# RRr89/Shared_SIMD_Scan

Measured on AMD Instinct MI355X. Metric: scanned values/sec + achieved HBM GB/s, 1e9 x 9-bit column (equality scan, bitmap + hit count out), higher is better.
Workload: dtype u32; 1 GPU; scan_eq ONE 1e+09x9bit column in 1 row-range shard(s) of <= 1000000000 rows, column=mod5, key=3; rows_total=1000000000, bits=9, parallelism=row-range shards x1

## Files before the change

shared_simd_scan_amd/csrc/kernels/scan.hpp:

```cpp
#pragma once

#include "tile.hpp"

namespace mi355 {

template <int C, int VPL> struct TileCtx {
    using G = ScanGeom<C, VPL>;
    uint64_t n, ntiles, nfull, data_bytes;
    uint32_t llc_inv, llc_lim;
    __device__ __forceinline__ TileCtx(uint64_t n_, uint32_t llc_inv_ = 0, uint32_t llc_lim_ = 0) : n(n_), llc_inv(llc_inv_), llc_lim(llc_lim_)
    {
        ntiles = (n + G::TILE_VALUES - 1) / G::TILE_VALUES;
        nfull = n / G::TILE_VALUES;
        data_bytes = (n * C + 7) / 8;
    }
    template <int AUX> __device__ __forceinline__ void issue(const uint8_t *packed, uint64_t t, uint8_t *lds_wave, int lane) const
    {
        if constexpr (AUX != 0) {
            if (llc_inv != 0 && (uint32_t)((t * G::TILE_BYTES) >> kLlcGranuleShift) * llc_inv <= llc_lim) {
                issue_as<0>(packed, t, lds_wave, lane);
                return;
            }
        }
        issue_as<AUX>(packed, t, lds_wave, lane);
    }
    template <int AUX> __device__ __forceinline__ void issue_as(const uint8_t *packed, uint64_t t, uint8_t *lds_wave, int lane) const
    {
        const uint8_t *src = packed + t * G::TILE_BYTES;
        if (t < nfull)
            dma_tile_full<G::TILE_BYTES, AUX>(src, lds_wave, lane);
        else
            dma_tile_partial<G::TILE_BYTES, AUX>(src, data_bytes - t * G::TILE_BYTES, lds_wave, lane);
    }
    __device__ __forceinline__ uint32_t finish_tail(uint64_t t, uint32_t (&v)[VPL / 32], uint8_t *dst, uint64_t byte_stride, int lane,
                                                    bool store = true) const
    {
        const int64_t left = (int64_t)(n - t * G::TILE_VALUES) - (int64_t)lane * VPL;
        const int valid = left >= VPL ? VPL : (left <= 0 ? 0 : (int)left);
        const int nbytes = (valid + 7) / 8;
        uint32_t cnt = 0;
#pragma unroll
        for (int j = 0; j < VPL / 32; j++) {
            v[j] &= tail_mask(valid, j);
            cnt += __builtin_popcount(v[j]);
#pragma unroll
            for (int b = 0; b < 4; b++)
                if (store && 4 * j + b < nbytes) dst[(uint64_t)(4 * j + b) * byte_stride] = (uint8_t)(v[j] >> (8 * b));
        }
        return cnt;
    }
};

template <int C, int VPL, int K> constexpr int burst_occ()
{
    using G = ScanGeom<C, VPL>;
    constexpr int mask_bytes = (K * G::BITMAP_BYTES + 1023) / 1024 * 1024;
    constexpr int table = narrow_k<C>() ? (1 << (narrow_k<C>() * C)) : 16;
    constexpr int lds = (160 * 1024) / (4 * (G::LDS_BYTES + mask_bytes) + table + 64);
    constexpr int cap = narrow_k<C>() ? 4 : 8;
    return lds > cap ? cap : (lds < 1 ? 1 : lds);
}

template <int C, int MODE, int AUX_, int VPL, int K>
__global__ __launch_bounds__(kBlockThreads, (burst_occ<C, VPL, K>())) void scan_burst_kernel(ScanArgs a)
{
    using G = ScanGeom<C, VPL>;
    static_assert(MODE == kModeEq || MODE == kModeRange, "MODE");
    constexpr int WORDS = G::WORDS;
    constexpr int AUX = AUX_ & 15;
    constexpr int NTS = store_policy_of(AUX_);
    __shared__ __attribute__((aligned(16))) uint8_t lds[kWavesPerBlock][G::LDS_BYTES];
    constexpr int LK = narrow_k<C>();
    __shared__ __attribute__((aligned(16))) uint8_t nlut[LK ? (1 << (LK * C)) : 16];
    constexpr int MASK_DMA = (K * G::BITMAP_BYTES + 1023) / 1024;
    __shared__ __attribute__((aligned(16))) uint8_t mlds[kWavesPerBlock][MASK_DMA * 1024];

    const int lane = threadIdx.x & 63;
    const int wave = __builtin_amdgcn_readfirstlane(threadIdx.x >> 6);
    uint8_t *lds_wave = lds[wave];
    uint8_t *mlds_wave = mlds[wave];
    const TileCtx<C, VPL> tc(a.n, a.llc_inv, a.llc_lim);
    const uint64_t nchunks = (tc.ntiles + K - 1) / K;
    const uint64_t stride = (uint64_t)gridDim.x * kWavesPerBlock;
    uint64_t chunk = (uint64_t)blockIdx.x * kWavesPerBlock + wave;

    uint32_t key[2] = {a.key[0], a.key[1]};
    uint32_t hits = 0;
    uint8_t *const out_lane = a.out + lane * (WORDS * 4);
    const bool store = a.out != nullptr;
    const uint8_t *const mask = a.and_mask;
    const uint32_t mop = a.mask_op, inv = a.invert;
    auto combine = [mop](uint32_t r, uint32_t m) -> uint32_t {
        return mop == 0 ? (r & m) : mop == 1 ? (r | m) : mop == 2 ? (r ^ m) : (m & ~r);
    };

    uint32_t res[K][WORDS];
    uint64_t pend_chunk = 0;
    int pend_n = 0;

    if (chunk < nchunks) tc.template issue<AUX>(a.packed, chunk * K, lds_wave, lane);
    if constexpr (LK > 0) {
        constexpr uint32_t fmask = (1u << C) - 1u;
        for (uint32_t e = threadIdx.x; e < (1u << (LK * C)); e += kBlockThreads) {
            uint32_t m = 0;
#pragma unroll
            for (int j = 0; j < LK; j++) {
                const uint32_t f = (e >> (j * C)) & fmask;
                const bool hit = (MODE == kModeRange) ? (f - key[0]) <= key[1] : f == key[0];
                m |= (hit ? 1u : 0u) << j;
            }
            nlut[e] = (uint8_t)m;
        }
        __syncthreads();
    }

    while (chunk < nchunks) {
        const uint64_t tfirst = chunk * K;
        int nfull_here = 0;
#pragma unroll
        for (int k = 0; k < K; k++) {
            const uint64_t tile = tfirst + k;
            if (tile < tc.ntiles) {
                asm volatile("s_waitcnt vmcnt(0)" ::: "memory");
                uint32_t w[G::LANE_DWORDS];
                read_lane_data<C, VPL>(lds_wave, lane, w);
                uint32_t mcur[WORDS];
                if (k > 0 && mask) {
#pragma unroll
                    for (int j = 0; j < WORDS; j++) mcur[j] = ((const uint32_t *)(mlds_wave + k * G::BITMAP_BYTES + lane * (WORDS * 4)))[j];
                }
                asm volatile("s_waitcnt lgkmcnt(0)" ::: "memory");
                if (k == 0) {
                    if (pend_n && store) {
                        uint8_t *dst = out_lane + pend_chunk * K * G::BITMAP_BYTES;
#pragma unroll
                        for (int q = 0; q < K; q++)
                            if (q < pend_n) store_words<WORDS, NTS>(dst + q * G::BITMAP_BYTES, res[q]);
                    }
                    pend_n = 0;
                    if (mask) {
                        const uint64_t mbytes = (tc.nfull > tfirst ? (tc.nfull - tfirst < K ? tc.nfull - tfirst : K) : 0) * G::BITMAP_BYTES;
                        const uint8_t *src = mask + tfirst * G::BITMAP_BYTES;
#pragma unroll
                        for (int q = 0; q < MASK_DMA; q++) {
                            const uint32_t o = q * 1024 + lane * 16;
                            if (o < mbytes) __builtin_amdgcn_global_load_lds(MI355_GPTR(src + o), MI355_LPTR(mlds_wave + q * 1024), 16, 0, 0);
                        }
                    }
                }
                const uint64_t next = (k + 1 < K && tile + 1 < tc.ntiles) ? tile + 1 : (chunk + stride) * K;
                const bool have_next = next < tc.ntiles && (k + 1 < K || chunk + stride < nchunks);
                if (have_next) tc.template issue<AUX>(a.packed, next, lds_wave, lane);
                uint32_t r1[1][WORDS];
                if constexpr (LK > 0) {
                    decode_words_narrow<C, VPL, LK, 0, G::LANE_DWORDS>(w, r1, nlut);
                } else {
                    const uint32_t key8[kMaxKeysPerPass] = {key[0], key[1], 0, 0, 0, 0, 0, 0};
                    decode_words<C, VPL, 0, 1, MODE, G::LANE_DWORDS>(w, r1, key8);
                }
#pragma unroll
                for (int j = 0; j < WORDS; j++) r1[0][j] ^= inv;
                if (tile < tc.nfull) {
                    if (mask) {
                        if (k == 0) {
                            if (have_next && next < tc.nfull)
                                asm volatile("s_waitcnt vmcnt(%0)" ::"n"(G::DMA_INSTRS) : "memory");
                            else
                                asm volatile("s_waitcnt vmcnt(0)" ::: "memory");
#pragma unroll
                            for (int j = 0; j < WORDS; j++) mcur[j] = ((const uint32_t *)(mlds_wave + lane * (WORDS * 4)))[j];
                            asm volatile("s_waitcnt lgkmcnt(0)" ::: "memory");
                        }
#pragma unroll
                        for (int j = 0; j < WORDS; j++) r1[0][j] = combine(r1[0][j], mcur[j]);
                    }
#pragma unroll
                    for (int j = 0; j < WORDS; j++) {
                        hits += __builtin_popcount(r1[0][j]);
                        res[k][j] = r1[0][j];
                    }
                    nfull_here = k + 1;
                } else {
                    if (mask) {
                        const uint8_t *mp = mask + tile * G::BITMAP_BYTES + lane * (WORDS * 4);
                        const int64_t left = (int64_t)(tc.n - tile * G::TILE_VALUES) - (int64_t)lane * VPL;
                        const int nbytes = left <= 0 ? 0 : (int)((left >= VPL ? VPL : left) + 7) / 8;
#pragma unroll
                        for (int j = 0; j < WORDS; j++) {
                            uint32_t m = 0;
#pragma unroll
                            for (int b = 0; b < 4; b++)
                                if (4 * j + b < nbytes) m |= (uint32_t)mp[4 * j + b] << (8 * b);
                            r1[0][j] = combine(r1[0][j], m);
                        }
                    }
                    hits += tc.finish_tail(tile, r1[0], out_lane + tile * G::BITMAP_BYTES, 1, lane, store);
                }
            }
        }
        pend_chunk = chunk;
        pend_n = nfull_here;
        chunk += stride;
    }
    if (pend_n && store) {
        uint8_t *dst = out_lane + pend_chunk * K * G::BITMAP_BYTES;
#pragma unroll
        for (int q = 0; q < K; q++)
            if (q < pend_n) store_words<WORDS, NTS>(dst + q * G::BITMAP_BYTES, res[q]);
    }
    if (a.hits) hits_add(a, 0, wave_sum(hits), lane);
    hits_finalize(a, 1, lane);
}

template <int C, int AUX_, int VPL>
__global__ __launch_bounds__(kBlockThreads, (burst_occ<C, VPL, 1>() > 1 ? burst_occ<C, VPL, 1>() / 2 : 1)) void scan2_kernel(ScanArgs a)
{
    using G = ScanGeom<C, VPL>;
    constexpr int WORDS = G::WORDS;
    constexpr int AUX = AUX_ & 15;
    constexpr int NTS = store_policy_of(AUX_);
    __shared__ __attribute__((aligned(16))) uint8_t lds[kWavesPerBlock][2][G::LDS_BYTES];

    const int lane = threadIdx.x & 63;
    const int wave = __builtin_amdgcn_readfirstlane(threadIdx.x >> 6);
    uint8_t *lds1 = lds[wave][0], *lds2 = lds[wave][1];
    const TileCtx<C, VPL> tc(a.n);
    const uint64_t stride = (uint64_t)gridDim.x * kWavesPerBlock;
    uint64_t tile = (uint64_t)blockIdx.x * kWavesPerBlock + wave;
    const uint32_t k1[kMaxKeysPerPass] = {a.key[0], a.key[1], 0, 0, 0, 0, 0, 0};
    const uint32_t k2[kMaxKeysPerPass] = {a.key2[0], a.key2[1], 0, 0, 0, 0, 0, 0};
    const uint32_t inv1 = a.invert, inv2 = a.invert2, mop = a.mask_op;
    auto combine = [mop](uint32_t p2, uint32_t p1) -> uint32_t {
        return mop == 0 ? (p2 & p1) : mop == 1 ? (p2 | p1) : mop == 2 ? (p2 ^ p1) : (p1 & ~p2);
    };
    uint32_t hits = 0;
    uint8_t *const out_lane = a.out + lane * (WORDS * 4);
    const bool store = a.out != nullptr;
    uint32_t res[WORDS];
    uint64_t prev = ~0ull;

    auto issue = [&](uint64_t t) {
        tc.template issue<AUX>(a.packed, t, lds1, lane);
        tc.template issue<AUX>(a.packed2, t, lds2, lane);
    };
    if (tile < tc.ntiles) issue(tile);
    while (tile < tc.ntiles) {
        asm volatile("s_waitcnt vmcnt(0)" ::: "memory");
        uint32_t w1[G::LANE_DWORDS], w2[G::LANE_DWORDS];
        read_lane_data<C, VPL>(lds1, lane, w1);
        read_lane_data<C, VPL>(lds2, lane, w2);
        asm volatile("s_waitcnt lgkmcnt(0)" ::: "memory");
        if (prev != ~0ull && store) store_words<WORDS, NTS>(out_lane + prev * G::BITMAP_BYTES, res);
        const uint64_t next = tile + stride;
        if (next < tc.ntiles) issue(next);
        uint32_t r1[1][WORDS], r2[1][WORDS];
        decode_words<C, VPL, 0, 1, kModeRange, G::LANE_DWORDS>(w1, r1, k1);
        decode_words<C, VPL, 0, 1, kModeRange, G::LANE_DWORDS>(w2, r2, k2);
#pragma unroll
        for (int j = 0; j < WORDS; j++) res[j] = combine(r2[0][j] ^ inv2, r1[0][j] ^ inv1);
        if (tile < tc.nfull) {
#pragma unroll
            for (int j = 0; j < WORDS; j++) hits += __builtin_popcount(res[j]);
            prev = tile;
        } else {
            hits += tc.finish_tail(tile, res, out_lane + tile * G::BITMAP_BYTES, 1, lane, store);
            prev = ~0ull;
        }
        tile = next;
    }
    if (prev != ~0ull && store) store_words<WORDS, NTS>(out_lane + prev * G::BITMAP_BYTES, res);
    if (a.hits) hits_add(a, 0, wave_sum(hits), lane);
    hits_finalize(a, 1, lane);
}

__device__ __forceinline__ void transpose4x4_bytes(const uint32_t (&r)[4], uint32_t (&c)[4])
{
    const uint32_t t0 = __builtin_amdgcn_perm(r[1], r[0], 0x05010400u);
    const uint32_t t1 = __builtin_amdgcn_perm(r[1], r[0], 0x07030602u);
    const uint32_t t2 = __builtin_amdgcn_perm(r[3], r[2], 0x05010400u);
    const uint32_t t3 = __builtin_amdgcn_perm(r[3], r[2], 0x07030602u);
    c[0] = __builtin_amdgcn_perm(t2, t0, 0x05040100u);
    c[1] = __builtin_amdgcn_perm(t2, t0, 0x07060302u);
    c[2] = __builtin_amdgcn_perm(t3, t1, 0x05040100u);
    c[3] = __builtin_amdgcn_perm(t3, t1, 0x07060302u);
}

}
```

shared_simd_scan_amd/csrc/kernels/tile.hpp:

```cpp
#pragma once

#include <hip/hip_runtime.h>
#include <stdint.h>

namespace mi355 {

typedef uint32_t u32x4 __attribute__((ext_vector_type(4)));
typedef uint32_t u32x2 __attribute__((ext_vector_type(2)));

#define MI355_GPTR(p) ((const __attribute__((address_space(1))) void *)(p))
#define MI355_LPTR(p) ((__attribute__((address_space(3))) void *)(p))

constexpr int kWavesPerBlock = 4;
constexpr int kBlockThreads = kWavesPerBlock * 64;
constexpr int kMaxKeysPerPass = 8;
constexpr int kMaxKeys = 1024;

template <int C, int VPL> struct ScanGeom {
    static_assert(VPL == 32 || VPL == 64 || VPL == 128, "VPL");
    static constexpr int WORDS = VPL / 32;
    static constexpr int LANE_DWORDS = VPL * C / 32;
    static constexpr int LANE_BYTES = LANE_DWORDS * 4;
    static constexpr int TILE_VALUES = 64 * VPL;
    static constexpr int TILE_BYTES = 64 * LANE_BYTES;
    static constexpr int DMA_INSTRS = (TILE_BYTES + 1023) / 1024;
    static constexpr int LDS_BYTES = DMA_INSTRS * 1024;
    static constexpr int BITMAP_BYTES = TILE_VALUES / 8;
    static constexpr int OCC_LDS = (160 * 1024) / (4 * LDS_BYTES + 64);
    static constexpr int OCC = OCC_LDS >= 8 ? 8 : (OCC_LDS < 1 ? 1 : OCC_LDS);
};

enum ScanMode { kModeEq = 0, kModeRange = 1, kModeShared = 2 };

template <int C> constexpr int narrow_k() { return C == 1 ? 8 : (C <= 3 ? 4 : (C <= 5 ? 3 : (C <= 7 ? 2 : 0))); }

template <int C, int VPL, int MODE> constexpr int scan_occ()
{
    constexpr int lds = ScanGeom<C, VPL>::OCC;
    if (MODE != 2 && C <= 7) {
        const int with_table = (160 * 1024) / (4 * ScanGeom<C, VPL>::LDS_BYTES + (1 << (narrow_k<C>() * C)) + 64);
        return with_table > 4 ? 4 : (with_table < 1 ? 1 : with_table);
    }
    return MODE == 2 ? (lds > 4 ? 4 : lds) : lds;
}

constexpr int scan_vpl(int C, int MODE)
{
    if (MODE == kModeShared) return 64;
    return C <= 16 ? 128 : 64;
}

struct ScanArgs {
    const uint8_t *packed;
    uint64_t n;
    uint8_t *out;
    uint64_t out_stride;
    unsigned long long *hits;
    unsigned long long *scratch;
    const int32_t *keys_dev;
    uint32_t key[kMaxKeysPerPass];
    uint32_t nkeys;
    uint32_t layout;
    const uint8_t *and_mask;
    uint32_t invert;
    uint32_t mask_op;
    uint32_t flags;
    const uint8_t *packed2;
    uint32_t key2[2];
    uint32_t invert2;
    unsigned long long *tile_state;
    uint64_t *rowids;
    uint64_t capacity;
    uint64_t first_row;
    uint32_t llc_d;
    uint32_t llc_inv, llc_lim;
};
constexpr int kLlcGranuleShift = 16;
inline void llc_set(ScanArgs &a, uint32_t d)
{
    a.llc_d = d;
    a.llc_inv = 0;
    a.llc_lim = 0;
    if (d == 0) return;
    uint32_t inv = d;
    for (int i = 0; i < 5; i++) inv *= 2u - d * inv;
    a.llc_inv = inv;
    a.llc_lim = 0xffffffffu / d;
}

template <int TILE_BYTES, int AUX>
__device__ __forceinline__ void dma_tile_full(const uint8_t *src, uint8_t *lds_wave, int lane)
{
    constexpr int N = (TILE_BYTES + 1023) / 1024;
#pragma unroll
    for (int j = 0; j < N; j++) {
        if ((j + 1) * 1024 <= TILE_BYTES) {
            __builtin_amdgcn_global_load_lds(MI355_GPTR(src + j * 1024 + lane * 16), MI355_LPTR(lds_wave + j * 1024), 16,
                                             0, AUX);
        } else if (lane * 16 < TILE_BYTES - j * 1024) {
            __builtin_amdgcn_global_load_lds(MI355_GPTR(src + j * 1024 + lane * 16), MI355_LPTR(lds_wave + j * 1024), 16,
                                             0, AUX);
        }
    }
}

template <int TILE_BYTES, int AUX>
__device__ __forceinline__ void dma_tile_partial(const uint8_t *src, uint64_t bytes_left, uint8_t *lds_wave, int lane)
{
    constexpr int N = (TILE_BYTES + 1023) / 1024;
#pragma unroll
    for (int j = 0; j < N; j++) {
        uint32_t o = j * 1024 + lane * 16;
        if (o < TILE_BYTES && o < bytes_left) {
            __builtin_amdgcn_global_load_lds(MI355_GPTR(src + o), MI355_LPTR(lds_wave + j * 1024), 16, 0, AUX);
        }
    }
}

template <int BIT, int LEN, int NW> __device__ __forceinline__ uint32_t extract_at(const uint32_t (&w)[NW])
{
    constexpr int d = BIT >> 5;
    constexpr int s = BIT & 31;
    if constexpr (LEN == 32 && s == 0) {
        return w[d];
    } else if constexpr (s + LEN <= 32) {
        return __builtin_amdgcn_ubfe(w[d], s, LEN);
    } else {
        return __builtin_amdgcn_alignbit(w[d + 1], w[d], s) & (LEN == 32 ? 0xffffffffu : ((1u << (LEN & 31)) - 1u));
    }
}

template <int C, int K, int NW> __device__ __forceinline__ uint32_t extract(const uint32_t (&w)[NW])
{
    constexpr int bit = K * C;
    constexpr int d = bit >> 5;
    constexpr int s = bit & 31;
    if constexpr (C == 32) {
        return w[d];
    } else if constexpr (s + C <= 32) {
        return __builtin_amdgcn_ubfe(w[d], s, C);
    } else {
        return __builtin_amdgcn_alignbit(w[d + 1], w[d], s) & ((1u << C) - 1u);
    }
}


__device__ __forceinline__ void push_eq8(uint32_t (&acc)[8], uint32_t x, const uint32_t (&key)[kMaxKeysPerPass])
{
    unsigned long long m0, m1, m2, m3, m4, m5, m6, m7;
    asm("v_cmp_eq_u32_e64 %8, %17, %16\n\t"
        "v_cmp_eq_u32_e64 %9, %18, %16\n\t"
        "v_cmp_eq_u32_e64 %10, %19, %16\n\t"
        "v_cmp_eq_u32_e64 %11, %20, %16\n\t"
        "v_cmp_eq_u32_e64 %12, %21, %16\n\t"
        "v_cmp_eq_u32_e64 %13, %22, %16\n\t"
        "v_cmp_eq_u32_e64 %14, %23, %16\n\t"
        "v_cmp_eq_u32_e64 %15, %24, %16\n\t"
        "v_addc_co_u32_e64 %0, %8, %0, %0, %8\n\t"
        "v_addc_co_u32_e64 %1, %9, %1, %1, %9\n\t"
        "v_addc_co_u32_e64 %2, %10, %2, %2, %10\n\t"
        "v_addc_co_u32_e64 %3, %11, %3, %3, %11\n\t"
        "v_addc_co_u32_e64 %4, %12, %4, %4, %12\n\t"
        "v_addc_co_u32_e64 %5, %13, %5, %5, %13\n\t"
        "v_addc_co_u32_e64 %6, %14, %6, %6, %14\n\t"
        "v_addc_co_u32_e64 %7, %15, %7, %7, %15"
        : "+v"(acc[0]), "+v"(acc[1]), "+v"(acc[2]), "+v"(acc[3]), "+v"(acc[4]), "+v"(acc[5]), "+v"(acc[6]), "+v"(acc[7]),
          "=&s"(m0), "=&s"(m1), "=&s"(m2), "=&s"(m3), "=&s"(m4), "=&s"(m5), "=&s"(m6), "=&s"(m7)
        : "v"(x), "s"(key[0]), "s"(key[1]), "s"(key[2]), "s"(key[3]), "s"(key[4]), "s"(key[5]), "s"(key[6]), "s"(key[7]));
}

template <int MODE> __device__ __forceinline__ void push1(uint32_t &a0, uint32_t x0, uint32_t k0, uint32_t k1)
{
    if constexpr (MODE == 1) {
        uint32_t t;
        asm("v_subrev_u32_e32 %1, %3, %2\n\t"
            "v_cmp_ge_u32_e32 vcc, %4, %1\n\t"
            "v_addc_co_u32_e32 %0, vcc, %0, %0, vcc"
            : "+v"(a0), "=&v"(t)
            : "v"(x0), "s"(k0), "s"(k1)
            : "vcc");
    } else {
        asm("v_cmp_eq_u32_e32 vcc, %2, %1\n\t"
            "v_addc_co_u32_e32 %0, vcc, %0, %0, vcc"
            : "+v"(a0)
            : "v"(x0), "s"(k0)
            : "vcc");
    }
}

template <int MODE>
__device__ __forceinline__ void push2(uint32_t &a0, uint32_t &a1, uint32_t x0, uint32_t x1, uint32_t k0, uint32_t k1)
{
    unsigned long long m0, m1;
    if constexpr (MODE == 1) {
        uint32_t t0, t1;
        asm("v_subrev_u32_e32 %4, %8, %6\n\t"
            "v_subrev_u32_e32 %5, %8, %7\n\t"
            "v_cmp_ge_u32_e64 %2, %9, %4\n\t"
            "v_cmp_ge_u32_e64 %3, %9, %5\n\t"
            "s_nop 0\n\t"
            "v_addc_co_u32_e64 %0, %2, %0, %0, %2\n\t"
            "v_addc_co_u32_e64 %1, %3, %1, %1, %3"
            : "+v"(a0), "+v"(a1), "=&s"(m0), "=&s"(m1), "=&v"(t0), "=&v"(t1)
            : "v"(x0), "v"(x1), "s"(k0), "s"(k1));
    } else {
        asm("v_cmp_eq_u32_e64 %2, %6, %4\n\t"
            "v_cmp_eq_u32_e64 %3, %6, %5\n\t"
            "s_nop 0\n\t"
            "v_addc_co_u32_e64 %0, %2, %0, %0, %2\n\t"
            "v_addc_co_u32_e64 %1, %3, %1, %1, %3"
            : "+v"(a0), "+v"(a1), "=&s"(m0), "=&s"(m1)
            : "v"(x0), "v"(x1), "s"(k0));
    }
}

template <int MODE>
__device__ __forceinline__ void push4(uint32_t &a0, uint32_t &a1, uint32_t &a2, uint32_t &a3, uint32_t x0, uint32_t x1,
                                      uint32_t x2, uint32_t x3, uint32_t k0, uint32_t k1)
{
    unsigned long long m0, m1, m2, m3;
    if constexpr (MODE == 1) {
        uint32_t t0, t1, t2, t3;
        asm("v_subrev_u32_e32 %8, %16, %12\n\t"
            "v_subrev_u32_e32 %9, %16, %13\n\t"
            "v_subrev_u32_e32 %10, %16, %14\n\t"
            "v_subrev_u32_e32 %11, %16, %15\n\t"
            "v_cmp_ge_u32_e64 %4, %17, %8\n\t"
            "v_cmp_ge_u32_e64 %5, %17, %9\n\t"
            "v_cmp_ge_u32_e64 %6, %17, %10\n\t"
            "v_cmp_ge_u32_e64 %7, %17, %11\n\t"
            "v_addc_co_u32_e64 %0, %4, %0, %0, %4\n\t"
            "v_addc_co_u32_e64 %1, %5, %1, %1, %5\n\t"
            "v_addc_co_u32_e64 %2, %6, %2, %2, %6\n\t"
            "v_addc_co_u32_e64 %3, %7, %3, %3, %7"
            : "+v"(a0), "+v"(a1), "+v"(a2), "+v"(a3), "=&s"(m0), "=&s"(m1), "=&s"(m2), "=&s"(m3), "=&v"(t0), "=&v"(t1),
              "=&v"(t2), "=&v"(t3)
            : "v"(x0), "v"(x1), "v"(x2), "v"(x3), "s"(k0), "s"(k1));
    } else {
        asm("v_cmp_eq_u32_e64 %4, %12, %8\n\t"
            "v_cmp_eq_u32_e64 %5, %12, %9\n\t"
            "v_cmp_eq_u32_e64 %6, %12, %10\n\t"
            "v_cmp_eq_u32_e64 %7, %12, %11\n\t"
            "v_addc_co_u32_e64 %0, %4, %0, %0, %4\n\t"
            "v_addc_co_u32_e64 %1, %5, %1, %1, %5\n\t"
            "v_addc_co_u32_e64 %2, %6, %2, %2, %6\n\t"
            "v_addc_co_u32_e64 %3, %7, %3, %3, %7"
            : "+v"(a0), "+v"(a1), "+v"(a2), "+v"(a3), "=&s"(m0), "=&s"(m1), "=&s"(m2), "=&s"(m3)
            : "v"(x0), "v"(x1), "v"(x2), "v"(x3), "s"(k0));
    }
}


template <int C, int VPL, int K, int MODE, int NW>
__device__ __forceinline__ void decode_step1(const uint32_t (&w)[NW], uint32_t (&res)[1][VPL / 32], uint32_t k0, uint32_t k1)
{
    if constexpr (VPL == 128) {
        push4<MODE>(res[0][0], res[0][1], res[0][2], res[0][3], extract<C, K, NW>(w), extract<C, 32 + K, NW>(w),
                    extract<C, 64 + K, NW>(w), extract<C, 96 + K, NW>(w), k0, k1);
    } else if constexpr (VPL == 64) {
        push2<MODE>(res[0][0], res[0][1], extract<C, K, NW>(w), extract<C, 32 + K, NW>(w), k0, k1);
    } else {
        push1<MODE>(res[0][0], extract<C, K, NW>(w), k0, k1);
    }
    if constexpr (K > 0) decode_step1<C, VPL, K - 1, MODE, NW>(w, res, k0, k1);
}

template <int C, int J, int K, int NW>
__device__ __forceinline__ void decode_step8(const uint32_t (&w)[NW], uint32_t (&acc)[8], const uint32_t (&key)[kMaxKeysPerPass])
{
    push_eq8(acc, extract<C, 32 * J + K, NW>(w), key);
    if constexpr (K > 0) decode_step8<C, J, K - 1, NW>(w, acc, key);
}

template <int C, int VPL, int J, int NW>
__device__ __forceinline__ void decode_words8(const uint32_t (&w)[NW], uint32_t (&res)[8][VPL / 32],
                                              const uint32_t (&key)[kMaxKeysPerPass])
{
    uint32_t acc[8];
#pragma unroll
    for (int q = 0; q < 8; q++) acc[q] = 0;
    decode_step8<C, J, 31, NW>(w, acc, key);
#pragma unroll
    for (int q = 0; q < 8; q++) res[q][J] = acc[q];
    if constexpr (J + 1 < VPL / 32) decode_words8<C, VPL, J + 1, NW>(w, res, key);
}

template <int C, int VPL, int J, int NK, int MODE, int NW>
__device__ __forceinline__ void decode_words(const uint32_t (&w)[NW], uint32_t (&res)[NK][VPL / 32],
                                             const uint32_t (&key)[kMaxKeysPerPass])
{
    if constexpr (NK == 8) {
        decode_words8<C, VPL, 0, NW>(w, res, key);
    } else {
#pragma unroll
        for (int j = 0; j < VPL / 32; j++) res[0][j] = 0;
        decode_step1<C, VPL, 31, MODE, NW>(w, res, key[0], key[1]);
    }
}

template <int C, int VPL>
__device__ __forceinline__ void read_lane_data(const uint8_t *lds_wave, int lane, uint32_t (&w)[VPL * C / 32])
{
    using G = ScanGeom<C, VPL>;
    if constexpr (VPL == 128) {
        const u32x4 *p = (const u32x4 *)(lds_wave + lane * G::LANE_BYTES);
#pragma unroll
        for (int q = 0; q < C; q++) {
            u32x4 v = p[q];
            w[4 * q + 0] = v.x;
            w[4 * q + 1] = v.y;
            w[4 * q + 2] = v.z;
            w[4 * q + 3] = v.w;
        }
    } else if constexpr (VPL == 64) {
        const u32x2 *p = (const u32x2 *)(lds_wave + lane * G::LANE_BYTES);
#pragma unroll
        for (int q = 0; q < C; q++) {
            u32x2 v = p[q];
            w[2 * q + 0] = v.x;
            w[2 * q + 1] = v.y;
        }
    } else {
        const uint32_t *p = (const uint32_t *)(lds_wave + lane * G::LANE_BYTES);
#pragma unroll
        for (int q = 0; q < C; q++) w[q] = p[q];
    }
}

__device__ __forceinline__ uint32_t wave_inclusive_scan(uint32_t x)
{
    uint32_t r = x;
    r += (uint32_t)__builtin_amdgcn_update_dpp(0, (int)x, 0x111, 0xf, 0xf, false);
    r += (uint32_t)__builtin_amdgcn_update_dpp(0, (int)x, 0x112, 0xf, 0xf, false);
    r += (uint32_t)__builtin_amdgcn_update_dpp(0, (int)x, 0x113, 0xf, 0xf, false);
    r += (uint32_t)__builtin_amdgcn_update_dpp(0, (int)r, 0x114, 0xf, 0xe, false);
    r += (uint32_t)__builtin_amdgcn_update_dpp(0, (int)r, 0x118, 0xf, 0xc, false);
    r += (uint32_t)__builtin_amdgcn_update_dpp(0, (int)r, 0x142, 0xa, 0xf, false);
    r += (uint32_t)__builtin_amdgcn_update_dpp(0, (int)r, 0x143, 0xc, 0xf, false);
    return r;
}

__device__ __forceinline__ uint32_t wave_sum(uint32_t v)
{
    return (uint32_t)__builtin_amdgcn_readlane((int)wave_inclusive_scan(v), 63);
}

__device__ __forceinline__ uint32_t tail_mask(int valid, int J)
{
    int v = valid - 32 * J;
    return v >= 32 ? 0xffffffffu : (v <= 0 ? 0u : ((1u << v) - 1u));
}

struct __attribute__((packed, aligned(1))) Unaligned64 { uint32_t lo, hi; };
__device__ __forceinline__ void store8_unaligned(uint8_t *dst, uint32_t lo, uint32_t hi)
{
    Unaligned64 v;
    v.lo = lo;
    v.hi = hi;
    *(Unaligned64 *)dst = v;
}

constexpr int store_policy_of(int aux) { return (aux & 32) ? 2 : ((aux & 16) ? 1 : 0); }

template <int WORDS, int NT = 0> __device__ __forceinline__ void store_words(uint8_t *dst, const uint32_t (&v)[WORDS])
{
    if constexpr (WORDS == 4) {
        u32x4 t = {v[0], v[1], v[2], v[3]};
        if constexpr (NT == 2) {
            asm volatile("global_store_dwordx4 %0, %1, off sc1" ::"v"(dst), "v"(t) : "memory");
        } else if constexpr (NT == 1) __builtin_nontemporal_store(t, (u32x4 *)dst); else *(u32x4 *)dst = t;
    } else if constexpr (WORDS == 2) {
        u32x2 t = {v[0], v[1]};
        if constexpr (NT == 2) {
            asm volatile("global_store_dwordx2 %0, %1, off sc1" ::"v"(dst), "v"(t) : "memory");
        } else if constexpr (NT == 1) __builtin_nontemporal_store(t, (u32x2 *)dst); else *(u32x2 *)dst = t;
    } else {
        if constexpr (NT) __builtin_nontemporal_store(v[0], (uint32_t *)dst); else *(uint32_t *)dst = v[0];
    }
}

constexpr int kHitSlots = 64;
constexpr int kDoneGroups = 16;
constexpr int kScratchWords = kHitSlots * kMaxKeys + 8 + kDoneGroups * 16;
constexpr int kScratchDone = kHitSlots * kMaxKeys;
constexpr int kScratchGroupDone = kScratchDone + 8;

__device__ __forceinline__ void hits_add(const ScanArgs &a, uint32_t k, uint32_t wave_total, int lane)
{
    if (lane == 0 && wave_total)
        __hip_atomic_fetch_add(a.scratch + (blockIdx.x % kHitSlots) * kMaxKeys + k, (unsigned long long)wave_total,
                               __ATOMIC_RELAXED, __HIP_MEMORY_SCOPE_AGENT);
}

__device__ __forceinline__ void hits_finalize(const ScanArgs &a, uint32_t P, int lane)
{
    if (!a.hits) return;
    __shared__ uint32_t s_last;
    asm volatile("s_waitcnt vmcnt(0)" ::: "memory");
    __syncthreads();
    if (threadIdx.x == 0) {
        const uint32_t g = blockIdx.x % kDoneGroups;
        const uint32_t in_group = (gridDim.x - g + kDoneGroups - 1) / kDoneGroups;
        const uint32_t ngroups = gridDim.x < (unsigned)kDoneGroups ? gridDim.x : (unsigned)kDoneGroups;
        unsigned long long *const gdone = a.scratch + kScratchGroupDone + g * 16;
        uint32_t last = 0;
        if (__hip_atomic_fetch_add(gdone, 1ull, __ATOMIC_RELAXED, __HIP_MEMORY_SCOPE_AGENT) == (unsigned long long)in_group - 1) {
            __hip_atomic_store(gdone, 0ull, __ATOMIC_RELAXED, __HIP_MEMORY_SCOPE_AGENT);
            last = __hip_atomic_fetch_add(a.scratch + kScratchDone, 1ull, __ATOMIC_RELAXED, __HIP_MEMORY_SCOPE_AGENT) == (unsigned long long)ngroups - 1;
        }
        s_last = last;
    }
    __syncthreads();
    if (s_last) {
        const uint32_t nslots = gridDim.x < (unsigned)kHitSlots ? gridDim.x : (unsigned)kHitSlots;
        if (P <= 16u) {
            for (uint32_t k = threadIdx.x >> 6; k < P; k += kBlockThreads / 64) {
                const unsigned long long v = (uint32_t)lane < nslots
                                                 ? __hip_atomic_exchange(a.scratch + (uint32_t)lane * kMaxKeys + k, 0ull, __ATOMIC_RELAXED, __HIP_MEMORY_SCOPE_AGENT)
                                                 : 0ull;
                const unsigned long long lo = wave_sum((uint32_t)(v & 0xffffffull)), mid = wave_sum((uint32_t)((v >> 24) & 0xffffffull)),
                                         hi = wave_sum((uint32_t)(v >> 48));
                if (lane == 0) a.hits[k] = lo + (mid << 24) + (hi << 48);
            }
            if (threadIdx.x == 0) __hip_atomic_store(a.scratch + kScratchDone, 0ull, __ATOMIC_RELAXED, __HIP_MEMORY_SCOPE_AGENT);
            return;
        }
        for (uint32_t k = threadIdx.x; k < P; k += kBlockThreads) {
            unsigned long long v = 0;
#pragma unroll 8
            for (uint32_t sl = 0; sl < nslots; sl++)
                v += __hip_atomic_exchange(a.scratch + sl * kMaxKeys + k, 0ull, __ATOMIC_RELAXED, __HIP_MEMORY_SCOPE_AGENT);
            a.hits[k] = v;
        }
        if (threadIdx.x == 0) __hip_atomic_store(a.scratch + kScratchDone, 0ull, __ATOMIC_RELAXED, __HIP_MEMORY_SCOPE_AGENT);
    }
}

__device__ __forceinline__ void block_hits_clear(uint32_t *s_hits)
{
    for (uint32_t k = threadIdx.x; k < (uint32_t)kMaxKeys; k += kBlockThreads) s_hits[k] = 0;
}
__device__ __forceinline__ void block_hits_add8(uint32_t *s_hits, uint32_t kbase, uint32_t P, const uint32_t (&cnt)[8], int lane)
{
    uint32_t p0 = cnt[0] | (cnt[1] << 16), p1 = cnt[2] | (cnt[3] << 16), p2 = cnt[4] | (cnt[5] << 16), p3 = cnt[6] | (cnt[7] << 16);
    p0 = wave_sum(p0);
    p1 = wave_sum(p1);
    p2 = wave_sum(p2);
    p3 = wave_sum(p3);
    if (lane == 0) {
        const uint32_t v[8] = {p0 & 0xffff, p0 >> 16, p1 & 0xffff, p1 >> 16, p2 & 0xffff, p2 >> 16, p3 & 0xffff, p3 >> 16};
#pragma unroll
        for (int q = 0; q < 8; q++)
            if (kbase + q < P && v[q]) atomicAdd(&s_hits[kbase + q], v[q]);
    }
}

__device__ __forceinline__ void block_hits_flush(const ScanArgs &a, uint32_t *s_hits, uint32_t P)
{
    __syncthreads();
    for (uint32_t k = threadIdx.x; k < P; k += blockDim.x) {
        const uint32_t v = s_hits[k];
        if (v)
            __hip_atomic_fetch_add(a.scratch + (blockIdx.x % kHitSlots) * kMaxKeys + k, (unsigned long long)v, __ATOMIC_RELAXED,
                                   __HIP_MEMORY_SCOPE_AGENT);
    }
}

template <int C, int LK, int J, int GI, int NW>
__device__ __forceinline__ void narrow_step(const uint32_t (&w)[NW], uint32_t &acc, const uint8_t *table)
{
    constexpr int FIRST = LK * GI;
    constexpr int LEN = (32 - FIRST) < LK ? (32 - FIRST) : LK;
    uint32_t m = table[extract_at<(32 * J + FIRST) * C, LEN * C, NW>(w)];
    if constexpr (LEN < LK) m &= (1u << LEN) - 1u;
    acc = (acc << LEN) | m;
    if constexpr (GI > 0) narrow_step<C, LK, J, GI - 1, NW>(w, acc, table);
}

template <int C, int VPL, int LK, int J, int NW>
__device__ __forceinline__ void decode_words_narrow(const uint32_t (&w)[NW], uint32_t (&res)[1][VPL / 32], const uint8_t *table)
{
    uint32_t acc = 0;
    narrow_step<C, LK, J, (32 + LK - 1) / LK - 1, NW>(w, acc, table);
    res[0][J] = acc;
    if constexpr (J + 1 < VPL / 32) decode_words_narrow<C, VPL, LK, J + 1, NW>(w, res, table);
}

}
```

shared_simd_scan_amd/csrc/width_group.hip:

```cpp
#include <type_traits>

#include "dispatch.hpp"
#include "kernels.hpp"
#include "launch_util.hpp"
#include "shared_plan.hpp"

#ifndef MI355_WLO
#error "compile with -DMI355_WLO=<first width> -DMI355_WHI=<last width> -DMI355_GROUP=<index>"
#endif

namespace mi355 {

namespace {

inline int scan_bpc(int occ_bpc, int tile_bytes, const LaunchReq &r)
{
    const int want = scan_want_bpc(tile_bytes, r.max_blocks_per_cu);
    return want < occ_bpc ? want : occ_bpc;
}

constexpr int burst_k(int c) { return (c == 5 || c == 6 || (c >= 9 && c <= 16)) ? 4 : 1; }

constexpr int kLlcAutoMiB = 205;
inline uint32_t llc_divisor(const LaunchReq &r, uint64_t column_bytes, uint64_t bitmap_bytes)
{
    if (r.llc_resident_mib == 0 || (r.dma_aux & 15) == 0) return 0;
    if (bitmap_bytes > (768ull << 20)) return 0;
    const bool automatic = r.llc_resident_mib < 0;
    if (automatic && !r.llc_repeat) return 0;
    const uint64_t budget = (uint64_t)(automatic ? kLlcAutoMiB : r.llc_resident_mib) << 20;
    if (budget <= bitmap_bytes) return 0;
    const uint64_t resident = budget - bitmap_bytes;
    if (resident >= column_bytes) return automatic ? 0 : 1;
    const uint64_t d = ((column_bytes + resident - 1) / resident) | 1u;
    return d > 0x7fffffu ? 0 : (uint32_t)d;
}

template <int C, int MODE> void launch_scan(const LaunchReq &r)
{
    constexpr int VPL = scan_vpl(C, MODE);
    using G = ScanGeom<C, VPL>;
    const uint64_t ntiles = (r.scan.n + G::TILE_VALUES - 1) / G::TILE_VALUES;
    const int policy = one_pass_store_policy(r.scan.n / 8, r.scan_nt_stores);
    ScanArgs a = r.scan;
    llc_set(a, llc_divisor(r, (r.scan.n * C + 7) / 8, (r.scan.out ? (r.scan.n + 7) / 8 : 0) + (r.scan.and_mask ? (r.scan.n + 7) / 8 : 0)));
    if (r.llc_d_out) *r.llc_d_out = (int)a.llc_d;
    auto go = [&](auto kc) {
        constexpr int K = decltype(kc)::value;
        static const int bpcK = blocks_per_cu(scan_burst_kernel<C, MODE, 34, VPL, K>);
        const dim3 grid(grid_for((ntiles + K - 1) / K, scan_bpc(bpcK, G::TILE_BYTES, r), r.num_cus));
        if (r.dma_aux == 0)
            MI355_LAUNCH(r, a.flags, (scan_burst_kernel<C, MODE, 0, VPL, K>), grid, dim3(kBlockThreads), 0, r.stream, a);
        else if (policy == 1)
            MI355_LAUNCH(r, a.flags, (scan_burst_kernel<C, MODE, 18, VPL, K>), grid, dim3(kBlockThreads), 0, r.stream, a);
        else if (policy == 2)
            MI355_LAUNCH(r, a.flags, (scan_burst_kernel<C, MODE, 34, VPL, K>), grid, dim3(kBlockThreads), 0, r.stream, a);
        else
            MI355_LAUNCH(r, a.flags, (scan_burst_kernel<C, MODE, 2, VPL, K>), grid, dim3(kBlockThreads), 0, r.stream, a);
    };
    if (burst_k(C) > 1 && r.scan_burst != 1)
        go(std::integral_constant<int, burst_k(C)>{});
    else
        go(std::integral_constant<int, 1>{});
}


template <auto Kernel> void launch_planned(const LaunchReq &r, const SharedPlan &p, int bpc, int max_dyn = 0)
{
    ScanArgs a = r.scan;
    a.flags |= p.set_flags;
    const uint64_t tile_values = 64 * (uint64_t)p.vpl;
    const dim3 grid(grid_for((a.n + tile_values - 1) / tile_values, bpc, r.num_cus));
    if (max_dyn > 0) allow_dynamic_lds<Kernel>(max_dyn, r.device);
    MI355_LAUNCH(r, a.flags, Kernel, grid, dim3(kBlockThreads), p.dyn_lds, r.stream, a);
}

template <auto Kernel, auto NtKernel> void launch_planned_nt(const LaunchReq &r, const SharedPlan &p, int bpc, int max_dyn = 0)
{
    p.store == 1 ? launch_planned<NtKernel>(r, p, bpc, max_dyn) : launch_planned<Kernel>(r, p, bpc, max_dyn);
}

template <int C, int VPL> void launch_pair(const LaunchReq &r, const SharedPlan &p)
{
    static const int occ = blocks_per_cu(shared_pair_kernel<C, 34, VPL>);
    launch_planned_nt<shared_pair_kernel<C, 34, VPL>, shared_pair_kernel<C, 18, VPL>>(r, p, p.want_bpc < occ ? p.want_bpc : occ);
}

template <int C, int VPL, int LINEAR> void launch_lut8(const LaunchReq &r, const SharedPlan &p)
{
    static const int occ = blocks_per_cu(shared_lut_kernel<C, 2, VPL, LINEAR, false>);
    const int bpc = p.want_bpc < occ ? p.want_bpc : occ;
    if (p.store == 2)
        launch_planned<shared_lut_kernel<C, 34, VPL, LINEAR, false>>(r, p, bpc);
    else
        launch_planned_nt<shared_lut_kernel<C, 2, VPL, LINEAR, false>, shared_lut_kernel<C, 18, VPL, LINEAR, false>>(r, p, bpc);
}

template <int C> void launch_shared(const LaunchReq &r, const SharedPlan &p)
{
    constexpr int VPL = kSharedVpl;
    constexpr bool kBigWidth = shared_big_width(C);
    constexpr int max_dyn = shared_max_dyn_lds<C>();
    const bool linear = r.scan.layout != 0;
    switch (p.form) {
    case kFormPair: p.vpl == 64 ? launch_pair<C, 64>(r, p) : launch_pair<C, scan_vpl(C, kModeEq)>(r, p); break;
    case kFormLut:
        if constexpr (C <= 12) {
            if (p.vpl == 128) {
                linear ? launch_lut8<C, 128, 1>(r, p) : launch_lut8<C, 128, 0>(r, p);
                break;
            }
        }
        linear ? launch_lut8<C, 64, 1>(r, p) : launch_lut8<C, 64, 0>(r, p);
        break;
    case kFormLinear3:
        with_rc_big<2, kBigWidth>(p.rc, p.big, [&](auto rc, auto big) {
            launch_planned<shared_linear3_kernel<C, 2, rc.value, big.value>>(r, p, p.want_bpc, (int)(kCuLds - linear3_fixed_lds<C>()));
        });
        break;
    case kFormLutMulti: launch_planned<shared_lut_kernel<C, 2, VPL, 1, true>>(r, p, p.want_bpc, max_dyn); break;
    case kFormLinearTwoRows: launch_planned<shared_linear_kernel<C, 2, 2>>(r, p, p.want_bpc, max_dyn); break;
    case kFormLinear: launch_planned<shared_linear_kernel<C, 2, 1>>(r, p, p.want_bpc, max_dyn); break;
    case kFormLinear2: launch_planned<shared_linear2_kernel<C, 2>>(r, p, p.want_bpc, max_dyn); break;
    case kFormWide3:
        with_rc_big<2, kBigWidth>(p.rc, p.big, [&](auto rc, auto big) {
            launch_planned_nt<shared_wide3_kernel<C, 2, rc.value, big.value>, shared_wide3_kernel<C, 18, rc.value, big.value>>(r, p, p.want_bpc, max_dyn);
        });
        break;
    case kFormWide2:
        with_rc_big<(C <= 10 ? 2 : 0), kBigWidth>(p.rc, p.big, [&](auto rc, auto big) {
            launch_planned_nt<shared_wide2_kernel<C, 2, VPL, rc.value, big.value>, shared_wide2_kernel<C, 18, VPL, rc.value, big.value>>(r, p, p.want_bpc,
                                                                                                                                       max_dyn);
        });
        break;
    case kFormWideLinear: launch_planned<shared_wide_kernel<C, 2, VPL, 1>>(r, p, p.want_bpc, max_dyn); break;
    case kFormWide: launch_planned_nt<shared_wide_kernel<C, 2, VPL, 0>, shared_wide_kernel<C, 18, VPL, 0>>(r, p, p.want_bpc, max_dyn); break;
    case kFormChain: {
        static const int occ = blocks_per_cu(shared_general_kernel<C, 2, VPL>);
        launch_planned<shared_general_kernel<C, 2, VPL>>(r, p, cap_bpc(occ, p.want_bpc));
        break;
    }
    default: break;
    }
}

template <int C> hipError_t launch_width(const LaunchReq &r)
{
    switch (r.op) {
    case kOpScanEq: launch_scan<C, kModeEq>(r); break;
    case kOpScanRange: launch_scan<C, kModeRange>(r); break;
    case kOpSharedScan: {
        const SharedPlan plan = plan_shared<C>(r);
        if (r.choice_out) *r.choice_out = plan.family;
        launch_shared<C>(r, plan);
        break;
    }
    case kOpScanIn: {
        constexpr int VPL = scan_vpl(C, kModeEq);
        using G = ScanGeom<C, VPL>;
        static const int bpc = blocks_per_cu(in_kernel<C, 2, VPL>);
        const uint64_t ntiles = (r.scan.n + G::TILE_VALUES - 1) / G::TILE_VALUES;
        int want = scan_bpc(bpc, G::TILE_BYTES, r);
        if (r.max_blocks_per_cu <= 0 && want < 2 && bpc >= 2) want = 2;
        const int ipol = one_pass_store_policy(r.scan.n / 8, r.scan_nt_stores);
        if (ipol == 2)
            MI355_LAUNCH(r, r.scan.flags, (in_kernel<C, 34, VPL>), dim3(grid_for(ntiles, want, r.num_cus)), dim3(kBlockThreads), 0, r.stream, r.scan);
        else if (ipol == 1)
            MI355_LAUNCH(r, r.scan.flags, (in_kernel<C, 18, VPL>), dim3(grid_for(ntiles, want, r.num_cus)), dim3(kBlockThreads), 0, r.stream, r.scan);
        else
            MI355_LAUNCH(r, r.scan.flags, (in_kernel<C, 2, VPL>), dim3(grid_for(ntiles, want, r.num_cus)), dim3(kBlockThreads), 0, r.stream, r.scan);
        break;
    }
    case kOpSelect: {
        constexpr int VPL = scan_vpl(C, kModeRange);
        using G = ScanGeom<C, VPL>;
        const uint64_t ntiles = (r.scan.n + G::TILE_VALUES - 1) / G::TILE_VALUES;
        const uint64_t nchunks = (ntiles + select_tiles(C) - 1) / select_tiles(C);
        const dim3 sgrid(grid_for(nchunks, 1, r.num_cus));
        if (r.select_single)
            MI355_LAUNCH(r, r.scan.flags, (select_kernel<C, kModeRange, VPL>), sgrid, dim3(kBlockThreads), 0, r.stream, r.scan);
        else
            MI355_LAUNCH(r, r.scan.flags, (select2_kernel<C, kModeRange, VPL>), sgrid, dim3(kSel2Waves * 64), 0, r.stream, r.scan);
        break;
    }
    case kOpScan2: {
        constexpr int VPL = scan_vpl(C, kModeRange);
        using G = ScanGeom<C, VPL>;
        static const int bpc = blocks_per_cu(scan2_kernel<C, 34, VPL>);
        const uint64_t ntiles = (r.scan.n + G::TILE_VALUES - 1) / G::TILE_VALUES;
        const dim3 grid(grid_for(ntiles, scan_bpc(bpc, 2 * G::TILE_BYTES, r), r.num_cus));
        const int policy = one_pass_store_policy(r.scan.n / 8, r.scan_nt_stores);
        if (policy == 1)
            MI355_LAUNCH(r, r.scan.flags, (scan2_kernel<C, 18, VPL>), grid, dim3(kBlockThreads), 0, r.stream, r.scan);
        else
            MI355_LAUNCH(r, r.scan.flags, (scan2_kernel<C, 34, VPL>), grid, dim3(kBlockThreads), 0, r.stream, r.scan);
        break;
    }
    case kOpDecompress: {
        static const int bpc = blocks_per_cu(decompress_kernel<C, 18>);
        const uint64_t ntiles = (r.decomp.n + DecompGeom<C>::TILE_VALUES - 1) / DecompGeom<C>::TILE_VALUES;
        const int want = bpc < 2 ? bpc : 2;
        const unsigned grid = grid_for(ntiles, r.max_blocks_per_cu > 0 ? cap_bpc(bpc, r.max_blocks_per_cu) : want, r.num_cus);
        if (r.dma_aux == 0)
            MI355_LAUNCH(r, 0, (decompress_kernel<C, 0>), dim3(grid), dim3(kBlockThreads), 0, r.stream, r.decomp);
        else if (r.dma_aux == 2)
            MI355_LAUNCH(r, 0, (decompress_kernel<C, 2>), dim3(grid), dim3(kBlockThreads), 0, r.stream, r.decomp);
        else if (r.dma_aux == 34)
            MI355_LAUNCH(r, 0, (decompress_kernel<C, 34>), dim3(grid), dim3(kBlockThreads), 0, r.stream, r.decomp);
        else
            MI355_LAUNCH(r, 0, (decompress_kernel<C, 18>), dim3(grid), dim3(kBlockThreads), 0, r.stream, r.decomp);
        break;
    }
    default:
        return hipErrorInvalidValue;
    }
    return launch_status(r);
}

}

hipError_t MI355_CAT(launch_group_, MI355_GROUP)(const LaunchReq &r)
{
    return launch_by_width<MI355_WLO, MI355_WHI>(r.c, r, [](auto c, const LaunchReq &q) { return launch_width<decltype(c)::value>(q); });
}

}
```

Before: 5277 billion values/s.

## Rebalance burst scan tail across all waves and use grouped ticket hit reduction

Restructures the burst scan's work schedule. Full rounds of K tiles per wave are now followed by a final partial round in which the leftover tiles are split evenly across all waves, instead of whole K-tile chunks being dealt out with a ragged last round. Grid sizing is now based on tile count rather than chunk count. Hit counting is replaced by a block-level LDS reduction plus a two-level grouped atomic ticket counter that packs count and arrival ticket into one 64-bit word, so fewer global atomics are issued per wave. This reduces tail imbalance and atomic traffic, at the cost of more complex index arithmetic and a __syncthreads at kernel exit.

```diff
diff --git a/shared_simd_scan_amd/csrc/kernels/scan.hpp b/shared_simd_scan_amd/csrc/kernels/scan.hpp
--- a/shared_simd_scan_amd/csrc/kernels/scan.hpp
+++ b/shared_simd_scan_amd/csrc/kernels/scan.hpp
@@ -80,9 +80,28 @@
     uint8_t *lds_wave = lds[wave];
     uint8_t *mlds_wave = mlds[wave];
     const TileCtx<C, VPL> tc(a.n, a.llc_inv, a.llc_lim);
-    const uint64_t nchunks = (tc.ntiles + K - 1) / K;
-    const uint64_t stride = (uint64_t)gridDim.x * kWavesPerBlock;
-    uint64_t chunk = (uint64_t)blockIdx.x * kWavesPerBlock + wave;
+    const uint32_t nwaves = gridDim.x * kWavesPerBlock;
+    const uint32_t wid = blockIdx.x * kWavesPerBlock + wave;
+    const uint64_t per_round = (uint64_t)nwaves * K;
+    uint64_t tfirst = (uint64_t)wid * K;
+    uint32_t cnt = 0;
+    const bool has_full = tc.ntiles >= per_round;
+    if (has_full) {
+        cnt = K;
+        tc.template issue<AUX>(a.packed, tfirst, lds_wave, lane);
+    }
+    const uint64_t rounds = (tc.ntiles >> 32) ? tc.ntiles / per_round : (uint64_t)((uint32_t)tc.ntiles / (uint32_t)per_round);
+    const uint32_t rem = (uint32_t)(tc.ntiles - rounds * per_round);
+    const uint32_t run = (rem + nwaves - 1) / nwaves;
+    const uint64_t last_first = rounds * per_round + (uint64_t)wid * run;
+    const uint32_t last_cnt = wid * run < rem ? (rem - wid * run < run ? rem - wid * run : run) : 0;
+    uint64_t full_left = has_full ? rounds - 1 : 0;
+    bool last_left = has_full && last_cnt > 0;
+    if (!has_full) {
+        tfirst = last_first;
+        cnt = last_cnt;
+        if (cnt) tc.template issue<AUX>(a.packed, tfirst, lds_wave, lane);
+    }
 
     uint32_t key[2] = {a.key[0], a.key[1]};
     uint32_t hits = 0;
@@ -95,10 +114,9 @@
     };
 
     uint32_t res[K][WORDS];
-    uint64_t pend_chunk = 0;
+    uint64_t pend_first = 0;
     int pend_n = 0;
 
-    if (chunk < nchunks) tc.template issue<AUX>(a.packed, chunk * K, lds_wave, lane);
     if constexpr (LK > 0) {
         constexpr uint32_t fmask = (1u << C) - 1u;
         for (uint32_t e = threadIdx.x; e < (1u << (LK * C)); e += kBlockThreads) {
@@ -114,13 +132,14 @@
         __syncthreads();
     }
 
-    while (chunk < nchunks) {
-        const uint64_t tfirst = chunk * K;
+    while (cnt) {
+        const uint64_t nfirst = full_left ? tfirst + per_round : last_first;
+        const uint32_t ncnt = full_left ? (uint32_t)K : (last_left ? last_cnt : 0u);
         int nfull_here = 0;
 #pragma unroll
         for (int k = 0; k < K; k++) {
             const uint64_t tile = tfirst + k;
-            if (tile < tc.ntiles) {
+            if ((uint32_t)k < cnt) {
                 asm volatile("s_waitcnt vmcnt(0)" ::: "memory");
                 uint32_t w[G::LANE_DWORDS];
                 read_lane_data<C, VPL>(lds_wave, lane, w);
@@ -132,14 +151,14 @@
                 asm volatile("s_waitcnt lgkmcnt(0)" ::: "memory");
                 if (k == 0) {
                     if (pend_n && store) {
-                        uint8_t *dst = out_lane + pend_chunk * K * G::BITMAP_BYTES;
+                        uint8_t *dst = out_lane + pend_first * G::BITMAP_BYTES;
 #pragma unroll
                         for (int q = 0; q < K; q++)
                             if (q < pend_n) store_words<WORDS, NTS>(dst + q * G::BITMAP_BYTES, res[q]);
                     }
                     pend_n = 0;
                     if (mask) {
-                        const uint64_t mbytes = (tc.nfull > tfirst ? (tc.nfull - tfirst < K ? tc.nfull - tfirst : K) : 0) * G::BITMAP_BYTES;
+                        const uint64_t mbytes = (tc.nfull > tfirst ? (tc.nfull - tfirst < cnt ? tc.nfull - tfirst : cnt) : 0) * G::BITMAP_BYTES;
                         const uint8_t *src = mask + tfirst * G::BITMAP_BYTES;
 #pragma unroll
                         for (int q = 0; q < MASK_DMA; q++) {
@@ -148,8 +167,9 @@
                         }
                     }
                 }
-                const uint64_t next = (k + 1 < K && tile + 1 < tc.ntiles) ? tile + 1 : (chunk + stride) * K;
-                const bool have_next = next < tc.ntiles && (k + 1 < K || chunk + stride < nchunks);
+                const bool in_run = (uint32_t)k + 1 < cnt;
+                const uint64_t next = in_run ? tile + 1 : nfirst;
+                const bool have_next = in_run || ncnt > 0;
                 if (have_next) tc.template issue<AUX>(a.packed, next, lds_wave, lane);
                 uint32_t r1[1][WORDS];
                 if constexpr (LK > 0) {
@@ -198,18 +218,22 @@
                 }
             }
         }
-        pend_chunk = chunk;
+        pend_first = tfirst;
         pend_n = nfull_here;
-        chunk += stride;
+        if (full_left)
+            full_left--;
+        else
+            last_left = false;
+        tfirst = nfirst;
+        cnt = ncnt;
     }
     if (pend_n && store) {
-        uint8_t *dst = out_lane + pend_chunk * K * G::BITMAP_BYTES;
+        uint8_t *dst = out_lane + pend_first * G::BITMAP_BYTES;
 #pragma unroll
         for (int q = 0; q < K; q++)
             if (q < pend_n) store_words<WORDS, NTS>(dst + q * G::BITMAP_BYTES, res[q]);
     }
-    if (a.hits) hits_add(a, 0, wave_sum(hits), lane);
-    hits_finalize(a, 1, lane);
+    hits_finish_single(a, hits, wave, lane);
 }
 
 template <int C, int AUX_, int VPL>
@@ -269,8 +293,7 @@
         tile = next;
     }
     if (prev != ~0ull && store) store_words<WORDS, NTS>(out_lane + prev * G::BITMAP_BYTES, res);
-    if (a.hits) hits_add(a, 0, wave_sum(hits), lane);
-    hits_finalize(a, 1, lane);
+    hits_finish_single(a, hits, wave, lane);
 }
 
 __device__ __forceinline__ void transpose4x4_bytes(const uint32_t (&r)[4], uint32_t (&c)[4])
diff --git a/shared_simd_scan_amd/csrc/kernels/tile.hpp b/shared_simd_scan_amd/csrc/kernels/tile.hpp
--- a/shared_simd_scan_amd/csrc/kernels/tile.hpp
+++ b/shared_simd_scan_amd/csrc/kernels/tile.hpp
@@ -436,6 +436,37 @@
     }
 }
 
+constexpr int kHitCountBits = 48;
+__device__ __forceinline__ void hits_finish_single(const ScanArgs &a, uint32_t lane_hits, int wave, int lane)
+{
+    if (!a.hits) return;
+    __shared__ uint32_t s_wave_hits[kWavesPerBlock];
+    const uint32_t wave_total = wave_sum(lane_hits);
+    if (lane == 0) s_wave_hits[wave] = wave_total;
+    __syncthreads();
+    if (threadIdx.x == 0) {
+        unsigned long long mine = 0;
+#pragma unroll
+        for (int w = 0; w < kWavesPerBlock; w++) mine += s_wave_hits[w];
+        constexpr unsigned long long kTicket = 1ull << kHitCountBits, kCount = kTicket - 1;
+        const uint32_t g = blockIdx.x % kDoneGroups;
+        const uint32_t in_group = (gridDim.x - g + kDoneGroups - 1) / kDoneGroups;
+        const uint32_t ngroups = gridDim.x < (unsigned)kDoneGroups ? gridDim.x : (unsigned)kDoneGroups;
+        unsigned long long *const gdone = a.scratch + kScratchGroupDone + g * 16;
+        unsigned long long *const top = a.scratch + kScratchDone;
+        const unsigned long long group = __hip_atomic_fetch_add(gdone, mine | kTicket, __ATOMIC_RELAXED, __HIP_MEMORY_SCOPE_AGENT) + (mine | kTicket);
+        if ((group >> kHitCountBits) == in_group) {
+            __hip_atomic_store(gdone, 0ull, __ATOMIC_RELAXED, __HIP_MEMORY_SCOPE_AGENT);
+            const unsigned long long add = (group & kCount) | kTicket;
+            const unsigned long long all = __hip_atomic_fetch_add(top, add, __ATOMIC_RELAXED, __HIP_MEMORY_SCOPE_AGENT) + add;
+            if ((all >> kHitCountBits) == ngroups) {
+                __hip_atomic_store(top, 0ull, __ATOMIC_RELAXED, __HIP_MEMORY_SCOPE_AGENT);
+                a.hits[0] = all & kCount;
+            }
+        }
+    }
+}
+
 __device__ __forceinline__ void block_hits_clear(uint32_t *s_hits)
 {
     for (uint32_t k = threadIdx.x; k < (uint32_t)kMaxKeys; k += kBlockThreads) s_hits[k] = 0;
diff --git a/shared_simd_scan_amd/csrc/width_group.hip b/shared_simd_scan_amd/csrc/width_group.hip
--- a/shared_simd_scan_amd/csrc/width_group.hip
+++ b/shared_simd_scan_amd/csrc/width_group.hip
@@ -48,7 +48,7 @@
     auto go = [&](auto kc) {
         constexpr int K = decltype(kc)::value;
         static const int bpcK = blocks_per_cu(scan_burst_kernel<C, MODE, 34, VPL, K>);
-        const dim3 grid(grid_for((ntiles + K - 1) / K, scan_bpc(bpcK, G::TILE_BYTES, r), r.num_cus));
+        const dim3 grid(grid_for(ntiles, scan_bpc(bpcK, G::TILE_BYTES, r), r.num_cus));
         if (r.dma_aux == 0)
             MI355_LAUNCH(r, a.flags, (scan_burst_kernel<C, MODE, 0, VPL, K>), grid, dim3(kBlockThreads), 0, r.stream, a);
         else if (policy == 1)
```

Result: slower. 5167 billion values/s (-2.1%).
